# iacopo97/Multimodal-SAM-Adapter

Measured on AMD Instinct MI355X. Metric: images/sec encoder fwd @1024x1024 RGB+LiDAR ViT-L, higher is better.
Workload: dtype split-operand MFMA: fp16 hi + e5m2 cross terms (h8c / h8 planes, ViT / interaction / up-conv GEMMs) fp16 hi/lo pairs x3 (TwinConvNeXt: f3 planes) and bf16 hi/lo x3 (neck, head); attention blocks with the rel-pos terms fused: every contraction on one fp16 MFMA (q, k, v, P rounded to fp16) in the bloc

## Files before the change

include/mmsa.h:

```cpp
#ifndef MMSA_H
#define MMSA_H
#include <stddef.h>
#include <stdint.h>
#ifdef __cplusplus
extern "C" {
#endif

#ifdef MMSA_BUILDING_LIBRARY
typedef hipStream_t mmsa_stream_t;
#else
typedef void* mmsa_stream_t;
#endif

#include "mmsa_version.h"
int mmsa_version(void);
const char* mmsa_last_error(void);

int mmsa_debug_poison_lds(unsigned pattern, mmsa_stream_t stream);
int mmsa_event_create(void** ev);
int mmsa_event_record(void* ev, mmsa_stream_t stream);
int mmsa_event_elapsed_ms(void* start, void* stop, float* ms);
int mmsa_event_destroy(void* ev);

enum { MMSA_ACT_NONE = 0, MMSA_ACT_GELU = 1, MMSA_ACT_RELU = 2, MMSA_ACT_RELU6 = 3, MMSA_ACT_HSWISH = 4, MMSA_ACT_SIGMOID = 5 };

enum { MMSA_DT_F32 = 0, MMSA_DT_F16 = 1, MMSA_DT_F64 = 2 };

enum { MMSA_FMT_B3 = 0, MMSA_FMT_H8 = 1, MMSA_FMT_H8C = 2, MMSA_FMT_F3 = 3, MMSA_FMT_W8 = 4  };

int mmsa_ms_deform_attn_forward(const void* value, const int64_t* spatial_shapes, const int64_t* level_start_index,
                                const void* sampling_loc, const void* attn_weight, void* out, int batch,
                                int spatial_size, int num_heads, int channels, int num_levels, int num_query,
                                int num_point, int im2col_step, int dtype, mmsa_stream_t stream);

int mmsa_ms_deform_attn_backward(const void* value, const int64_t* spatial_shapes, const int64_t* level_start_index,
                                 const void* sampling_loc, const void* attn_weight, const void* grad_output,
                                 void* grad_value, void* grad_sampling_loc, void* grad_attn_weight, int batch,
                                 int spatial_size, int num_heads, int channels, int num_levels, int num_query,
                                 int num_point, int im2col_step, int dtype, mmsa_stream_t stream);

int mmsa_msda_fused(const float* value, const int64_t* spatial_shapes, const int64_t* level_start_index,
                    const float* raw, long ldraw, const float* ref_points, float* out, long ldo,
                    uint16_t* out_planes, long ldop , int out_fmt , int batch,
                    int spatial_size, int num_heads, int channels, int num_levels, int num_query, int num_point,
                    float* clamp_max , mmsa_stream_t stream);

int mmsa_msda_fused_planes(const uint16_t* value_planes, long ldvp, int lo_bytes, const int64_t* spatial_shapes, const int64_t* level_start_index,
                           const float* raw, long ldraw, const float* ref_points, float* out, long ldo,
                           uint16_t* out_planes, long ldop, int out_fmt, int batch,
                           int spatial_size, int num_heads, int channels, int num_levels, int num_query, int num_point,
                           float* clamp_max, mmsa_stream_t stream);

int mmsa_rowstats_finalize(const float* rowstats, int rows, int strips, int D, float eps, float* mean_rstd, mmsa_stream_t stream);

int mmsa_zero_bytes(void* p, size_t bytes, mmsa_stream_t stream);
int mmsa_gemm_split3(const float* A, const uint16_t* Ap, long lda, long strideA,
                     const uint16_t* Wp, long strideW,
                     const float* bias, long strideBias, const float* colscale, const float* resid, long ldr,
                     long strideR, int resid_mod, float beta, float* C, long ldc, long strideC,
                     uint16_t* Cp, long ldcp, long strideCp, int M, int N, int K,
                     int batch, int act, float alpha, int out_mode, int ps_H, int ps_W, int ps_C, int fmt, int cp_fmt,
                     int max_grid, float* rowstats_out, const float* rownorm_mean_rstd, const float* rownorm_colsum, int flavour,
                     float* clamp_max , mmsa_stream_t stream);

int mmsa_convnext_mlp_fused(const uint16_t* Ap, long lda, long strideA, const uint16_t* W1p, long strideW1, const uint16_t* W2p,
                            long strideW2, const float* b1, const float* b2, const float* gamma, float* x, long ldx, long strideX,
                            int M, int C, int batch, int max_grid, int fmt,
                            float* clamp_max , mmsa_stream_t stream);

int mmsa_split_planes(const float* src, long ld, int rows, int cols, int cols_pad, uint16_t* planes, int kind,
                      float* clamp_max , mmsa_stream_t stream);

int mmsa_attention(const float* qkv, long ldq, const float* qkv_bias, const float* rp, float* out, long ldo, int B,
                   int H, int W, int heads, int head_dim, int window_size, float scale, mmsa_stream_t stream);
int mmsa_attention_planes(const uint16_t* qkv_planes, long ldq, const uint16_t* bias_planes, const float* rp,
                          uint16_t* out_planes, long ldo, int B, int H, int W, int heads, int head_dim,
                          int window_size, float scale, int out_fmt ,
                          int v_fmt ,
                          float* max_abs_logit , mmsa_stream_t stream);

int mmsa_relpos_bias(const float* qkv, long ldq, const float* Rh, const float* Rw, float* rp, int B, int H, int W,
                     int heads, int head_dim, int window_size, mmsa_stream_t stream);
int mmsa_relpos_bias_planes(const uint16_t* qkv_planes, long ldq, const float* Rh, const float* Rw,
                            float* rp, int B, int H, int W, int heads, int head_dim, int window_size, mmsa_stream_t stream);

int mmsa_layernorm_rows(const float* x, long ldx, const float* w, const float* b, float eps, float* y, long ldy,
                        float* y2, long ldy2, uint16_t* y_planes, long ldp ,
                        int rows, int C, int map_mode, int map_H, int map_W, int group_rows, long w_gstride, long y_gcol,
                        int y_wrap, int plane_fmt , float* clamp_max ,
                        mmsa_stream_t stream);

int mmsa_colstats(const float* x, long ldx, long strideB, const float* wrow, int B, int HW, int C, double* out,
                  int out_is_zero , mmsa_stream_t stream);

int mmsa_ffrm_finalize(const double* stats, int B, int HW, int C, float mean_w, float mean_b, const float* Wc,
                       const float* gn_w, const float* gn_b, float* mean_o, float* rstd_o, float* mult_o,
                       float* scratch , mmsa_stream_t stream);
int mmsa_lnhw_apply(const float* x, long ldx, const float* mean, const float* rstd, const float* mult, const float* w,
                    const float* bias, float* y, long ldy, int B, int HW, int C, mmsa_stream_t stream);

int mmsa_dwconv_nhwc(const float* x, long ldx, long xstrideB, const float* w, const float* bias, float* y, long ldy,
                     long ystrideB, uint16_t* y_planes, long ldp, long pstrideB , int planes_fmt ,
                     int B, int H, int W, int C, int k, int act,
                     int imgs_per_group ,
                     float* rowstats ,
                     float* clamp_max , mmsa_stream_t stream);
int mmsa_gconv_nhwc(const float* x, long ldx, const float* w, const float* bias, float* y, long ldy, int B, int H,
                    int W, int G, int cin_g, int cout_g, int k, int act, mmsa_stream_t stream);
int mmsa_gfe_qkv_conv(const float* x, long ldx, const float* w, float* y, long ldy, int B, int H, int W, int G, int cin_g, int cout_g,
                      int* covered, mmsa_stream_t stream);
int mmsa_dwpair_gate(const float* x, long ldx, const float* w, float* y, long ldy, uint16_t* y_planes, long ldp, int B, int H,
                     int W, int C, mmsa_stream_t stream);
int mmsa_im2col_nchw(const float* x, int B, int Ctot, int c0, int Cin, int H, int W, int p, float* out, int Kpad,
                     mmsa_stream_t stream);

long mmsa_gram_tn_scratch_bytes(int B, int P, int c);
int mmsa_gram_tn(const float* X, long ldx, const float* Y, long ldy, long strideB, double* G , int B, int P, int c,
                 int nblk, void* scratch, long scratch_bytes, mmsa_stream_t stream);
int mmsa_chanattn_build(const double* G, const double* sq, long sq_strideB, const double* sk, long sk_strideB,
                        const float* temp, const float* Wp, uint16_t* planes , int B, int c, int cpad,
                        int heads, mmsa_stream_t stream);
// ... 136 lines not shown
```

multimodal-sam-adapter_amd/csrc/mlp_fused.hip:

```cpp
#include "common.h"

#define MF_GLDS16(gptr, lptr)                                                                               \
  __builtin_amdgcn_global_load_lds((const __attribute__((address_space(1))) void*)(gptr),                   \
                                   (__attribute__((address_space(3))) void*)(lptr), 16, 0, 0)

struct MlpFusedArgs {
  const unsigned short* Ap; long lda; long strideA;
  const unsigned short* W1p; long strideW1;
  const unsigned short* W2p; long strideW2;
  const float* b1; const float* b2; const float* gamma;
  float* x; long ldx; long strideX;
  int M, batch;
  int ntiles, tiles_per_batch;
  float* clamp;
};

#define MF_C 96
#define MF_HID (4 * MF_C)
#define MF_AS_BYTES (3 * 16384)
#define MF_SLOT 24576
#define MF_RING_OFF MF_AS_BYTES
#define MF_HS_OFF (MF_RING_OFF + 3 * MF_SLOT)
#define MF_BS_OFF (MF_HS_OFF + 32768)
#define MF_LDS (MF_BS_OFF + 8192)

template <bool F16>
__global__ __launch_bounds__(512, 1) void mlp_fused_kernel(MlpFusedArgs a) {
  float cw_ = 0.f;
  constexpr int C = MF_C, HID = MF_HID;
  constexpr int NSTEP = 2 * (HID / 64);
  constexpr int NT = C / 32;
  extern __shared__ __attribute__((aligned(16))) unsigned char smem[];
  unsigned char* As = smem;
  unsigned char* Hs = smem + MF_HS_OFF;
  float* Bs = reinterpret_cast<float*>(smem + MF_BS_OFF);
  for (int i = threadIdx.x; i < a.batch * HID; i += 512) Bs[i] = a.b1[i];
  const int tid = threadIdx.x, lane = tid & 63;
  const int wave = __builtin_amdgcn_readfirstlane(tid >> 6);
  const int wm = wave >> 1, wn = wave & 1;
  const int l15 = lane & 15, g = lane >> 4;
  const int drow = lane >> 3;
  const int dp_even = ((lane & 7) ^ (drow >> 1)) * 8;
  const int fslot = g ^ ((l15 >> 1) & 7);
  const int frag_hi = l15 * 128 + fslot * 16;
  const int frag_lo = l15 * 128 + (fslot ^ 4) * 16;
  const long w1_off = (long)(8 * wave + drow) * (2 * C) + ((wave & 1) ? (dp_even ^ 32) : dp_even);
  int w2_kb[3], w2_dst[3];
  long w2_off[3];
#pragma unroll
  for (int i = 0; i < 3; ++i) {
    const int p = wave + 8 * i, kb2 = p / 12, q = p - 12 * kb2;
    w2_kb[i] = kb2;
    w2_dst[i] = kb2 * 12288 + q * 1024;
    w2_off[i] = (long)(8 * q + drow) * (2 * HID) + ((q & 1) ? (dp_even ^ 32) : dp_even);
  }

  auto tile_of = [&](int tile, int& bz, int& m0) { bz = tile / a.tiles_per_batch; m0 = (tile - bz * a.tiles_per_batch) * 128; };
  auto issue_a = [&](int tile) {
    int bz, m0;
    tile_of(tile, bz, m0);
    const unsigned short* Ab = a.Ap + (long)bz * a.strideA;
#pragma unroll
    for (int i = 0; i < 6; ++i) {
      const int p = wave + 8 * i, kb = p >> 4, q = p & 15;
      const int row = min(m0 + 8 * q + drow, a.M - 1);
      MF_GLDS16(Ab + (long)row * a.lda + kb * 64 + ((q & 1) ? (dp_even ^ 32) : dp_even), As + kb * 16384 + q * 1024);
    }
  };
  auto issue = [&](int t, const unsigned short* W1b, const unsigned short* W2b, int slot) {
    unsigned char* sb = smem + MF_RING_OFF + slot * MF_SLOT;
    const int j = t >> 1;
    if ((t & 1) == 0) {
#pragma unroll
      for (int kb = 0; kb < 3; ++kb) MF_GLDS16(W1b + (long)j * 64 * (2 * C) + w1_off + kb * 64, sb + kb * 8192 + wave * 1024);
    } else {
#pragma unroll
      for (int i = 0; i < 3; ++i) MF_GLDS16(W2b + w2_off[i] + (2 * j + w2_kb[i]) * 64, sb + w2_dst[i]);
    }
  };

  int slot_c = 0;
  int tile = blockIdx.x;
  if (tile < a.ntiles) issue_a(tile);
  for (; tile < a.ntiles; tile += gridDim.x) {
    int bz, m0;
    tile_of(tile, bz, m0);
    const unsigned short* W1b = a.W1p + (long)bz * a.strideW1;
    const unsigned short* W2b = a.W2p + (long)bz * a.strideW2;
    f32x4 acc_o[2][NT];
#pragma unroll
    for (int mi = 0; mi < 2; ++mi)
#pragma unroll
      for (int nj = 0; nj < NT; ++nj) acc_o[mi][nj] = (f32x4){0.f, 0.f, 0.f, 0.f};
    f32x4 acc_h[2][2];
    issue(0, W1b, W2b, slot_c);
    issue(1, W1b, W2b, slot_c == 2 ? 0 : slot_c + 1);

#pragma unroll 1
    for (int t = 0; t < NSTEP; ++t) {
      if (t + 1 < NSTEP) asm volatile("s_waitcnt vmcnt(3)" ::: "memory");
      else asm volatile("s_waitcnt vmcnt(0)" ::: "memory");
      asm volatile("s_waitcnt lgkmcnt(0)" ::: "memory");
      __syncthreads();
      const unsigned char* sb = smem + MF_RING_OFF + slot_c * MF_SLOT;
      const int pf_slot = slot_c == 0 ? 2 : slot_c - 1;
      const int j = t >> 1;
      if ((t & 1) == 0) {
#pragma unroll
        for (int mi = 0; mi < 2; ++mi)
#pragma unroll
          for (int ni = 0; ni < 2; ++ni) acc_h[mi][ni] = (f32x4){0.f, 0.f, 0.f, 0.f};
#pragma unroll
        for (int kb = 0; kb < 3; ++kb) {
          bf16x8 ah[2], al[2], wh[2], wl[2];
#pragma unroll
          for (int i = 0; i < 2; ++i) {
            ah[i] = *reinterpret_cast<const bf16x8*>(As + kb * 16384 + (wm * 32 + i * 16) * 128 + frag_hi);
            al[i] = *reinterpret_cast<const bf16x8*>(As + kb * 16384 + (wm * 32 + i * 16) * 128 + frag_lo);
            wh[i] = *reinterpret_cast<const bf16x8*>(sb + kb * 8192 + (wn * 32 + i * 16) * 128 + frag_hi);
            wl[i] = *reinterpret_cast<const bf16x8*>(sb + kb * 8192 + (wn * 32 + i * 16) * 128 + frag_lo);
          }
#pragma unroll
          for (int mi = 0; mi < 2; ++mi)
#pragma unroll
            for (int ni = 0; ni < 2; ++ni) {
              acc_h[mi][ni] = (F16 ? __builtin_amdgcn_mfma_f32_16x16x32_f16(__builtin_bit_cast(f16x8, wl[ni]), __builtin_bit_cast(f16x8, ah[mi]), acc_h[mi][ni], 0, 0, 0) : __builtin_amdgcn_mfma_f32_16x16x32_bf16(wl[ni], ah[mi], acc_h[mi][ni], 0, 0, 0));
              acc_h[mi][ni] = (F16 ? __builtin_amdgcn_mfma_f32_16x16x32_f16(__builtin_bit_cast(f16x8, wh[ni]), __builtin_bit_cast(f16x8, al[mi]), acc_h[mi][ni], 0, 0, 0) : __builtin_amdgcn_mfma_f32_16x16x32_bf16(wh[ni], al[mi], acc_h[mi][ni], 0, 0, 0));
              acc_h[mi][ni] = (F16 ? __builtin_amdgcn_mfma_f32_16x16x32_f16(__builtin_bit_cast(f16x8, wh[ni]), __builtin_bit_cast(f16x8, ah[mi]), acc_h[mi][ni], 0, 0, 0) : __builtin_amdgcn_mfma_f32_16x16x32_bf16(wh[ni], ah[mi], acc_h[mi][ni], 0, 0, 0));
            }
        }
        if (t + 2 < NSTEP) issue(t + 2, W1b, W2b, pf_slot);
        const float* b1p = Bs + bz * HID + j * 64 + wn * 32;
#pragma unroll
        for (int ni = 0; ni < 2; ++ni) {
          const float4 bb = *reinterpret_cast<const float4*>(b1p + ni * 16 + 4 * g);
#pragma unroll
          for (int mi = 0; mi < 2; ++mi) {
            float4 o = make_float4(acc_h[mi][ni][0] + bb.x, acc_h[mi][ni][1] + bb.y, acc_h[mi][ni][2] + bb.z, acc_h[mi][ni][3] + bb.w);
            o = gelu4(o);
            uint2 hh, ll;
            if constexpr (F16) { clamp_see(cw_, o); f3_split4(o, hh, ll); } else split4(o, hh, ll);
            const int row = wm * 32 + mi * 16 + l15;
            const int chunk = ni * 2 + (g >> 1);
            const int sw = (row >> 1) & 7;
            unsigned char* rb = Hs + wn * 16384 + row * 128 + (g & 1) * 8;
            *reinterpret_cast<uint2*>(rb + ((chunk ^ sw) << 4)) = hh;
            *reinterpret_cast<uint2*>(rb + (((chunk + 4) ^ sw) << 4)) = ll;
          }
        }
      } else {
#pragma unroll
        for (int kb2 = 0; kb2 < 2; ++kb2) {
          bf16x8 ah[2], al[2];
#pragma unroll
          for (int i = 0; i < 2; ++i) {
            ah[i] = *reinterpret_cast<const bf16x8*>(Hs + kb2 * 16384 + (wm * 32 + i * 16) * 128 + frag_hi);
            al[i] = *reinterpret_cast<const bf16x8*>(Hs + kb2 * 16384 + (wm * 32 + i * 16) * 128 + frag_lo);
          }
#pragma unroll
          for (int nj = 0; nj < NT; ++nj) {
            const bf16x8 wh = *reinterpret_cast<const bf16x8*>(sb + kb2 * 12288 + (wn * (C / 2) + nj * 16) * 128 + frag_hi);
            const bf16x8 wl = *reinterpret_cast<const bf16x8*>(sb + kb2 * 12288 + (wn * (C / 2) + nj * 16) * 128 + frag_lo);
#pragma unroll
            for (int mi = 0; mi < 2; ++mi) {
              acc_o[mi][nj] = (F16 ? __builtin_amdgcn_mfma_f32_16x16x32_f16(__builtin_bit_cast(f16x8, wl), __builtin_bit_cast(f16x8, ah[mi]), acc_o[mi][nj], 0, 0, 0) : __builtin_amdgcn_mfma_f32_16x16x32_bf16(wl, ah[mi], acc_o[mi][nj], 0, 0, 0));
              acc_o[mi][nj] = (F16 ? __builtin_amdgcn_mfma_f32_16x16x32_f16(__builtin_bit_cast(f16x8, wh), __builtin_bit_cast(f16x8, al[mi]), acc_o[mi][nj], 0, 0, 0) : __builtin_amdgcn_mfma_f32_16x16x32_bf16(wh, al[mi], acc_o[mi][nj], 0, 0, 0));
              acc_o[mi][nj] = (F16 ? __builtin_amdgcn_mfma_f32_16x16x32_f16(__builtin_bit_cast(f16x8, wh), __builtin_bit_cast(f16x8, ah[mi]), acc_o[mi][nj], 0, 0, 0) : __builtin_amdgcn_mfma_f32_16x16x32_bf16(wh, ah[mi], acc_o[mi][nj], 0, 0, 0));
            }
          }
        }
        if (t + 2 < NSTEP) issue(t + 2, W1b, W2b, pf_slot);
        else if (t == NSTEP - 1 && tile + (int)gridDim.x < a.ntiles) issue_a(tile + gridDim.x);
      }
      slot_c = slot_c == 2 ? 0 : slot_c + 1;
    }

    float* xb = a.x + (long)bz * a.strideX;
    const float* b2p = a.b2 + (long)bz * C + wn * (C / 2);
    const float* gp = a.gamma + (long)bz * C + wn * (C / 2);
#pragma unroll
    for (int nj = 0; nj < NT; ++nj) {
      const float4 bb = *reinterpret_cast<const float4*>(b2p + nj * 16 + 4 * g);
      const float4 gg = *reinterpret_cast<const float4*>(gp + nj * 16 + 4 * g);
#pragma unroll
      for (int mi = 0; mi < 2; ++mi) {
        const int m = m0 + wm * 32 + mi * 16 + l15;
        if (m < a.M) {
          float* px = xb + (long)m * a.ldx + wn * (C / 2) + nj * 16 + 4 * g;
          const float4 rr = *reinterpret_cast<const float4*>(px);
          float4 o;
          o.x = rr.x + gg.x * (acc_o[mi][nj][0] + bb.x);
          o.y = rr.y + gg.y * (acc_o[mi][nj][1] + bb.y);
          o.z = rr.z + gg.z * (acc_o[mi][nj][2] + bb.z);
          o.w = rr.w + gg.w * (acc_o[mi][nj][3] + bb.w);
          *reinterpret_cast<float4*>(px) = o;
        }
      }
    }
  }
  if constexpr (F16) clamp_report(a.clamp, cw_, MMSA_F3_MAX);
}

extern "C" int mmsa_convnext_mlp_fused(const unsigned short* Ap, long lda, long strideA, const unsigned short* W1p, long strideW1,
                                       const unsigned short* W2p, long strideW2, const float* b1, const float* b2, const float* gamma,
                                       float* x, long ldx, long strideX, int M, int C, int batch, int max_grid, int fmt, float* clamp_max, hipStream_t stream) {
  MMSA_CHECK_ARG(Ap && W1p && W2p && b1 && b2 && gamma && x && M > 0 && batch > 0, "convnext_mlp_fused: bad args");
  MMSA_CHECK_ARG(C == MF_C, "convnext_mlp_fused: C = %d not supported (%d)", C, MF_C);
  MMSA_CHECK_ARG(fmt == MMSA_FMT_B3 || fmt == MMSA_FMT_F3, "convnext_mlp_fused: planes format %d (bf16 hi/lo or f3)", fmt);
  MMSA_CHECK_ARG((long)batch * 4 * C <= 2048, "convnext_mlp_fused: batch * 4C = %ld > 2048 (bias staging)", (long)batch * 4 * C);
  MMSA_CHECK_ARG(lda >= 2L * C && (lda & 63) == 0 && (strideA & 63) == 0 && (strideW1 & 63) == 0 && (strideW2 & 63) == 0,
                 "convnext_mlp_fused: plane strides must be multiples of 64");
  MMSA_CHECK_ARG(((((uintptr_t)Ap) | ((uintptr_t)W1p) | ((uintptr_t)W2p)) & 127) == 0, "convnext_mlp_fused: planes must be 128-byte aligned");
  MMSA_CHECK_ARG(((((uintptr_t)x) | ((uintptr_t)b1) | ((uintptr_t)b2) | ((uintptr_t)gamma)) & 15) == 0 && (ldx & 3) == 0 && (strideX & 3) == 0 && ldx >= C,
                 "convnext_mlp_fused: fp32 pointers must be 16-byte aligned, ldx %% 4 == 0");
  MlpFusedArgs a;
  a.Ap = Ap; a.lda = lda; a.strideA = strideA; a.W1p = W1p; a.strideW1 = strideW1; a.W2p = W2p; a.strideW2 = strideW2;
  a.b1 = b1; a.b2 = b2; a.gamma = gamma; a.x = x; a.ldx = ldx; a.strideX = strideX; a.M = M; a.batch = batch; a.clamp = clamp_max;
  a.tiles_per_batch = cdiv(M, 128);
  a.ntiles = a.tiles_per_batch * batch;
  static MmsaPerDevice per_dev_ = {};
  const int num_cus = mmsa_per_device(per_dev_, [] {
    (void)hipFuncSetAttribute((const void*)mlp_fused_kernel<false>, hipFuncAttributeMaxDynamicSharedMemorySize, MF_LDS);
    (void)hipFuncSetAttribute((const void*)mlp_fused_kernel<true>, hipFuncAttributeMaxDynamicSharedMemorySize, MF_LDS);
  });
  const int cus = (max_grid > 0 && max_grid < num_cus) ? max_grid : num_cus;
  const int grid = a.ntiles < cus ? a.ntiles : cus;
  if (fmt == MMSA_FMT_F3) hipLaunchKernelGGL(mlp_fused_kernel<true>, dim3(grid), dim3(512), MF_LDS, stream, a);
  else hipLaunchKernelGGL(mlp_fused_kernel<false>, dim3(grid), dim3(512), MF_LDS, stream, a);
  MMSA_CHECK_LAUNCH("convnext_mlp_fused");
  return MMSA_OK;
}
```

multimodal-sam-adapter_amd/mmsa/backbone.py:

```python
import contextlib
import functools
import math
import os

import torch
import torch.nn as nn

from . import ops, pack
from .pack import PackPlan, _linear_resize_rows, fold_gfe_qkv
from .params import CONVNEXT_ARCH, build_tree

_VIT_DEFAULTS = dict(img_size=1024, patch_size=16, in_chans=3, embed_dim=1024, depth=24, mlp_ratio=4.0,
                     qkv_bias=True, use_abs_pos=True, use_rel_pos=True, rel_pos_zero_init=True, window_size=14,
                     global_attn_indexes=[5, 11, 17, 23], pretrained_size=1024, fix=False)


class OperandRangeError(RuntimeError):
    """A forward converted a value beyond the range of an fp16-based operand format (the clamp watch word, include/mmsa.h) and nothing is left to
    re-route: `range_fallback` is off, or the value is a q / k / v (or a qkv bias / rel-pos table entry) beyond +-65504 inside the attention kernels,
    which read fp16-based planes in every mode.  The outputs of that forward are invalid."""


class Workspace:

# ... 690 lines not shown
            for i in range(4):
                self._taps[f"twin{i}"] = tcat[i].clone()
        offs = [0, 0, sizes[1][0] * sizes[1][1], sizes[1][0] * sizes[1][1] + sizes[2][0] * sizes[2][1]]
        joins = []
        for i in range(4):
            sn = s_neck[i]
            sn.wait_event(ev_x[i])
            with torch.cuda.stream(sn):
                if i == 0:
                    self._neck_level(0, pk["neck"][0], tcat[0], B, sizes[0][0], sizes[0][1], chans[0], c1_out, 0, tcat_p[0])
                else:
                    self._neck_level(i, pk["neck"][i], tcat[i], B, sizes[i][0], sizes[i][1], chans[i], cbuf[offs[i]:], Nc * D, tcat_p[i])
                e = torch.cuda.Event()
                e.record(sn)
                joins.append(e)
        if not join:
            return joins
        for e in joins[1:]:
            main.wait_event(e)
        return joins[0]

    def _twin_batched(self, x, B, sizes, tcat, stage_events, tcat_p=None):
        pk, ws = self._packed, self._ws
        chans = self.channels
        st = pk["twin2"]
        t = "cnb_"
        h0, w0 = sizes[0]
        P0 = B * h0 * w0
        kp = st["stem"].kpad
        a = ws.get(t + "stem_a", 2 * P0, kp)
        for si in range(2):
            ops.im2col_nchw(x, 3 * si, 3, 4, a[si * P0:(si + 1) * P0])
        t0 = ws.get(t + "tmp", 2 * P0, chans[0])
        ops.gemm(a, st["stem"], t0, bias=st["stem_b"], batch=2, m=P0, stride_a=P0 * kp, stride_w=st["stem"].n * 2 * kp,
                 stride_bias=chans[0], stride_c=P0 * chans[0])
        cur = ws.get(t + "cur0", 2 * P0, chans[0])
        ops.layernorm(t0, st["stem_nw"], st["stem_nb"], 1e-6, cur, group_rows=P0, w_gstride=chans[0])
        for i in range(4):
            hh, wwd = sizes[i]
            P = B * hh * wwd
            c = chans[i]
            if i >= 1:
                ds = st["ds"][i - 1]
                cp = chans[i - 1]
                Pp = B * sizes[i - 1][0] * sizes[i - 1][1]
                pa = ws.planes(t + "patch", 2 * P, 4 * cp, fmt=ds["w"].fmt)
                ops.layernorm(cur, ds["nw"], ds["nb"], 1e-6, out_planes=pa, patchify=(sizes[i - 1][0], sizes[i - 1][1]),
                              group_rows=Pp, w_gstride=cp)
                cur = ws.get(t + f"cur{i}", 2 * P, c)
                ops.gemm(pa, ds["w"], cur, bias=ds["b"], batch=2, m=P, stride_a=P * 2 * pa.kpad, stride_w=ds["w"].n * 2 * ds["w"].kpad,
                         stride_bias=c, stride_c=P * c)
            d = ws.get(t + "tmp", 2 * P, c)
            wf = st["stages"][i][0]["pw1"].fmt
            n = ws.planes(t + "n", 2 * P, c, fmt=wf)
            hbuf = ws.planes(t + "h", 2 * P, 4 * c, fmt=st["stages"][i][0]["pw2"].fmt)
            fuse_mlp = ops.convnext_mlp_fused_supported(c) and bool(getattr(self, "fuse_convnext_mlp", True))
            fold = "pw1f" in st["stages"][i][0] and not fuse_mlp and hh % 8 == 0 and wwd % 8 == 0 and P >= 128
            if fold:
                rs = ws.get(t + "rs", 2 * P, 2 * (c // 64))
                mr = ws.get(t + "mr", 2 * P, 2)
            for blk in st["stages"][i]:
                if fold:
                    ops.dwconv(cur, blk["dw"], blk["dw_b"], None, 2 * B, hh, wwd, 7, imgs_per_group=B, out_planes=n, rowstats_out=rs)
                    ops.rowstats_finalize(rs, 2 * P, c, 1e-6, mr)
                    ops.gemm(n, blk["pw1f"], bias=blk["pw1_bf"], act="gelu", out_planes=hbuf, row_norm=(mr, blk["pw1_cs"]), batch=2, m=P,
                             stride_a=P * 2 * n.kpad, stride_w=blk["pw1f"].n * 2 * blk["pw1f"].kpad, stride_bias=4 * c, stride_cp=P * 2 * hbuf.kpad)
                    ops.gemm(hbuf, blk["pw2"], cur, bias=blk["pw2_b"], colscale=blk["gamma"], resid=cur, batch=2, m=P,
                             stride_a=P * 2 * hbuf.kpad, stride_w=blk["pw2"].n * 2 * blk["pw2"].kpad, stride_bias=c,
                             stride_r=P * c, stride_c=P * c)
                    continue
                ops.dwconv(cur, blk["dw"], blk["dw_b"], d, 2 * B, hh, wwd, 7, imgs_per_group=B)
                ops.layernorm(d, blk["nw"], blk["nb"], 1e-6, out_planes=n, group_rows=P, w_gstride=c)
                if fuse_mlp:
                    ops.convnext_mlp_fused(n, blk["pw1"], blk["pw2"], blk["pw1_b"], blk["pw2_b"], blk["gamma"], cur, P, batch=2,
                                           stride_a=P * 2 * n.kpad, stride_w1=blk["pw1"].n * 2 * blk["pw1"].kpad,
                                           stride_w2=blk["pw2"].n * 2 * blk["pw2"].kpad, stride_x=P * c)
                    continue
                ops.gemm(n, blk["pw1"], bias=blk["pw1_b"], act="gelu", out_planes=hbuf, batch=2, m=P, stride_a=P * 2 * n.kpad,
                         stride_w=blk["pw1"].n * 2 * blk["pw1"].kpad, stride_bias=4 * c, stride_cp=hbuf.batch_stride(P))
                ops.gemm(hbuf, blk["pw2"], cur, bias=blk["pw2_b"], colscale=blk["gamma"], resid=cur, batch=2, m=P,
                         stride_a=hbuf.batch_stride(P), stride_w=blk["pw2"].batch_stride(blk["pw2"].n), stride_bias=c,
                         stride_r=P * c, stride_c=P * c)
            nw, nb = st["out_norm"][i]
            ops.layernorm(cur, nw, nb, 1e-6, tcat[i], group_rows=P, w_gstride=c, y_gcol=c, y_wrap=True,
                          out_planes=tcat_p[i] if tcat_p is not None else None)
            ev = torch.cuda.Event()
            ev.record(torch.cuda.current_stream())
            stage_events.append(ev)

    def _neck_level(self, level, lv, t, B, h, w, c, out, out_stride_b, tp=None):
        ws = _Tagged(self._ws, f"nk{level}_")
        C = 2 * c
        HW = h * w
        P = B * HW
        gcat = ws.get("nk_g", P, C)
        lcat = ws.get("nk_l", P, C)
        pl_ok = tp is not None and c % 32 == 0
        gcat_p = ws.planes("nk_gp", P, C) if pl_ok else None
        lcat_p = ws.planes("nk_lp", P, C) if pl_ok else None
        n_st, n_g, n_st2 = B * 3 * 3 * c, B * c * c, B * 3 * C
        acc_blk = ws.get("nk_acc", 1, 2 * (n_st + n_g) + n_g + n_st2, dtype=torch.float64)
        ops.zero_(acc_blk[0, :2 * n_st + n_st2])
        gram_scr = ws.get("nk_gscr", 1, (ops.gram_tn_scratch_bytes(B, HW, c) + 3) // 4)
        acc_off = [0, 2 * n_st + n_st2]

        def acc_buf(rows, cols, gram=False):
            o = acc_off[int(gram)]
            acc_off[int(gram)] = o + rows * cols
            return acc_blk[0, o:o + rows * cols].view(rows, cols)
        for m in range(2):
            X = t[:, m * c:(m + 1) * c]
            gp = lv["gfe"][m]
            y = ws.get("nk_y", P, c)
            s = ws.get("nk_s", P, c)
            ops.layernorm(X, gp["nw"], gp["nb"], 1e-5, y, out2=s)
            q2 = ws.get("nk_q2", P, 3 * c)
            if not ("q12" in gp and getattr(self, "fuse_gfe_qkv", True) and ops.gfe_qkv(y, gp["q12"], q2, B, h, w, 32, c // 32, 3 * c // 32)):
                q1 = ws.get("nk_q1", P, 3 * c)
                ops.gconv(y, gp["q1"], None, q1, B, h, w, 32, c // 32, 3 * c // 32, 1)
                ops.gconv(q1, gp["q2"], None, q2, B, h, w, 32, 3 * c // 32, 3 * c // 32, 3)
            st = acc_buf(B * 3, 3 * c)
            ops.colstats(q2, HW * 3 * c, B, HW, st, out_is_zero=True)
            g = acc_buf(B * c, c, gram=True)
            ops.gram_tn(q2[:, :c], q2[:, c:2 * c], HW * 3 * c, g, B, HW, nblk=8, scratch=gram_scr)
# ... 125 lines not shown
```

multimodal-sam-adapter_amd/mmsa/lib.py:

```python
import ctypes
import os
from ctypes import c_char_p, c_double, c_float, c_int, c_long, c_void_p, POINTER

_HERE = os.path.dirname(os.path.abspath(__file__))
LIB_PATH = os.environ.get("MMSA_LIB") or os.path.join(_HERE, "libmmsa_hip.so")

if not os.path.exists(LIB_PATH):
    raise RuntimeError(
        f"{LIB_PATH} not found: the MI355X HIP library is required (no CPU/PyTorch fallback exists). "
        "Build it with: python multimodal-sam-adapter_amd/build.py")

import torch

_lib = ctypes.CDLL(LIB_PATH)

P = c_void_p
I = c_int
L = c_long
F = c_float

_PAINT_TAIL = [P, I, P, I, I, I, I, I, P, P, I, I, c_double, c_double, c_double, c_double, P, P]
SIGNATURES = {
    "mmsa_version": [],
    "mmsa_last_error": [],
    "mmsa_debug_poison_lds": [ctypes.c_uint, P],
    "mmsa_event_create": [POINTER(c_void_p)],
    "mmsa_event_record": [P, P],
    "mmsa_event_elapsed_ms": [P, P, POINTER(c_float)],
    "mmsa_event_destroy": [P],
    "mmsa_ms_deform_attn_forward": [P, P, P, P, P, P, I, I, I, I, I, I, I, I, I, P],
    "mmsa_ms_deform_attn_backward": [P, P, P, P, P, P, P, P, P, I, I, I, I, I, I, I, I, I, P],
    "mmsa_msda_fused": [P, P, P, P, L, P, P, L, P, L, I, I, I, I, I, I, I, I, P, P],
    "mmsa_msda_fused_planes": [P, L, I, P, P, P, L, P, P, L, P, L, I, I, I, I, I, I, I, I, P, P],
    "mmsa_gemm_split3": [P, P, L, L, P, L, P, L, P, P, L, L, I, F, P, L, L, P, L, L, I, I, I, I, I, F, I, I, I, I, I, I, I, P, P, P, I, P, P],
    "mmsa_convnext_mlp_fused": [P, L, L, P, L, P, L, P, P, P, P, L, L, I, I, I, I, I, P, P],
    "mmsa_rowstats_finalize": [P, I, I, I, F, P, P],
    "mmsa_zero_bytes": [P, ctypes.c_size_t, P],
    "mmsa_split_planes": [P, L, I, I, I, P, I, P, P],
    "mmsa_attention": [P, L, P, P, P, L, I, I, I, I, I, I, F, P],
    "mmsa_attention_planes": [P, L, P, P, P, L, I, I, I, I, I, I, F, I, I, P, P],
    "mmsa_relpos_bias": [P, L, P, P, P, I, I, I, I, I, I, P],
    "mmsa_relpos_bias_planes": [P, L, P, P, P, I, I, I, I, I, I, P],
    "mmsa_layernorm_rows": [P, L, P, P, F, P, L, P, L, P, L, I, I, I, I, I, I, L, L, I, I, P, P],
    "mmsa_colstats": [P, L, L, P, I, I, I, P, I, P],
    "mmsa_ffrm_finalize": [P, I, I, I, F, F, P, P, P, P, P, P, P, P],
    "mmsa_lnhw_apply": [P, L, P, P, P, P, P, P, L, I, I, I, P],
    "mmsa_dwconv_nhwc": [P, L, L, P, P, P, L, L, P, L, L, I, I, I, I, I, I, I, I, P, P, P],
    "mmsa_dwpair_gate": [P, L, P, P, L, P, L, I, I, I, I, P],
    "mmsa_gconv_nhwc": [P, L, P, P, P, L, I, I, I, I, I, I, I, I, P],
    "mmsa_gfe_qkv_conv": [P, L, P, P, L, I, I, I, I, I, I, POINTER(c_int), P],
    "mmsa_im2col_nchw": [P, I, I, I, I, I, I, I, P, I, P],
    "mmsa_gram_tn": [P, L, P, L, L, P, I, I, I, I, P, L, P],
    "mmsa_gram_tn_scratch_bytes": [I, I, I],
    "mmsa_chanattn_build": [P, P, L, P, L, P, P, P, I, I, I, I, P],
    "mmsa_gffm_build": [P, P, P, I, I, I, P],
    "mmsa_gelu_gate": [P, L, P, L, L, I, P],
    "mmsa_pool_hw": [P, L, P, L, I, I, I, I, P],
    "mmsa_ca_apply": [P, L, P, L, P, L, P, L, I, I, I, I, P],
    "mmsa_tail_fuse": [P, L, L, P, L, P, P, P, P, L, I, I, I, I, I, I, P],
    "mmsa_global_attention_planes": [P, L, P, P, P, L, I, I, I, I, I, F, I, I, P, P],
    "mmsa_window_attention_planes": [P, L, P, P, P, P, L, I, I, I, I, I, I, F, I, I, P, P],
    "mmsa_nchw_to_planes": [P, L, P, L, I, I, L, P],
    "mmsa_head_fuse": [P, P, I, I, P, I, I, P, I, I, L, P, P, P, L, P, L, I, I, I, I, I, P],
    "mmsa_tokens_to_nchw": [P, L, P, I, L, I, P],
    "mmsa_bilinear_accum_nchw": [P, L, I, I, I, I, P, I, I, I, I, I, I, P, I, P],
    "mmsa_div_count_nchw": [P, P, I, I, L, P],
    "mmsa_argmax_nchw": [P, P, I, I, L, P],
    "mmsa_crop_batch_nchw": [P, I, I, I, I, P, I, P, I, I, P],
    "mmsa_slide_argmax": [P, I, I, I, I, P, P, I, I, I, I, I, P, P],
    "mmsa_slide_argmax_resized": [P, I, I, I, I, P, P, I, I, I, I, I, I, I, I, I, P, P],
    "mmsa_softmax_flip_accum_nchw": [P, P, I, I, I, I, I, I, I, P],
    "mmsa_aug_argmax": [P, P, I, I, P, P, I, P, I, I, I, P, P],
    "mmsa_argmax_max_nchw": [P, P, P, I, I, L, P],
    "mmsa_slide_argmax_conf": [P, I, I, I, I, P, P, P, I, I, I, I, I, P, P],
    "mmsa_slide_argmax_resized_conf": [P, I, I, I, I, P, P, P, I, I, I, I, I, I, I, I, I, P, P],
    "mmsa_aug_argmax_conf": [P, P, I, I, P, P, I, P, P, I, I, I, P, P],
    "mmsa_preprocess_nhwc": [P, I, P, I, I, I, I, P, P, P, P, P, P, I, I, P],
    "mmsa_preprocess_crops": [P, I, P, I, I, I, I, P, P, P, P, P, I, I, P, I, P, I, I, P],
    "mmsa_preprocess_resize_nhwc": [P, I, P, I, I, I, I, P, P, P, P, P, P, I, I, I, I, P, P, P, P, I, P],
    "mmsa_preprocess_resize_crops": [P, I, P, I, I, I, I, P, P, P, P, P, I, I, P, I, P, I, I, I, I, P, P, P, P, I, P],
    "mmsa_eval_confusion_u8": [P, P, I, I, I, I, I, P, I, P, P, P, I, P, P],
    "mmsa_eval_calibration": [P, P, P, I, I, I, I, I, P, I, P, P, P, I, I, P, P],
    "mmsa_eval_selective": [P, P, P, I, I, I, I, I, P, I, P, P, P, I, I, P, P],
    "mmsa_abstain_u8": [P, P, L, I, I, P, P],
    "mmsa_slide_argmax_conf_t": [P, I, I, I, I, P, P, P, I, I, I, I, I, P, F, P],
    "mmsa_slide_argmax_resized_conf_t": [P, I, I, I, I, P, P, P, I, I, I, I, I, I, I, I, I, P, F, P],
    "mmsa_softmax_flip_accum_nchw_t": [P, P, I, I, I, I, I, I, I, F, P],
    "mmsa_temperature_sweep_nchw": [P, P, I, I, I, I, I, I, P, P, P, P, I, P, I, I, P, P],
# ... 49 lines not shown
```

multimodal-sam-adapter_amd/mmsa/ops.py:

```python
import ctypes

import os

import torch

from . import lib

ACT = {"none": 0, "gelu": 1, "relu": 2, "relu6": 3, "hswish": 4, "sigmoid": 5}

GEMM_PROFILE = None
CLAMP_WATCH = None
GEMM_MAX_GRID = 0
GEMM_FLAVOUR = 0
GEMM_SHAPES = None


def _event():
    ev = ctypes.c_void_p()
    lib.call("mmsa_event_create", ctypes.byref(ev))
    return ev


def collect_gemm_profile(prof):
    flops, ms = 0.0, 0.0
# ... 249 lines not shown


def gemm(a, w, out=None, bias=None, act="none", alpha=1.0, colscale=None, resid=None, beta=1.0, resid_mod=0,
         batch=1, stride_a=0, stride_w=0, stride_bias=0, stride_r=0, stride_c=0, m=None, pixel_shuffle=None,
         out_planes=None, stride_cp=0, rowstats_out=None, row_norm=None):
    fmt = w.fmt
    if isinstance(a, Planes):
        pap, ma, ka, lda = a.mat("A")
        pa = None
        if ka < w.kpad:
            raise RuntimeError(f"mmsa.gemm: A planes have {ka} columns but the packed weight expects K={w.kpad}")
        if a.fmt != w.afmt or a.weight or (w.fmt == FMT_H8 and not w.weight) or (w.fmt == FMT_H8C and w.weight):
            raise RuntimeError(f"mmsa.gemm: operand formats differ (A fmt {a.fmt}, W fmt {w.fmt} weight={w.weight})")
    elif fmt not in (FMT_B3, FMT_F3):
        raise RuntimeError("mmsa.gemm: h8 weights need A as h8 planes")
    else:
        pa, ma, ka, lda = _mat(a, "A")
        pap = None
        if ka < w.kpad and lda < w.kpad:
            raise RuntimeError(f"mmsa.gemm: A has {ka} columns (ld {lda}) but the packed weight expects K={w.kpad}")
    m = ma if m is None else m
    pc, ldc = None, 0
    if out is not None:
        pc, _, _, ldc = _mat(out, "C")
    pcp, ldcp = None, 0
    if out_planes is not None:
        pcp, _, _, ldcp = out_planes.mat("Cplanes")
    pr, ldr = None, 0
    if resid is not None:
        pr, _, _, ldr = _mat(resid, "resid")
    ps = pixel_shuffle or (0, 0, 0)
    prof = GEMM_PROFILE
    if prof is not None:
        e0, e1 = _event(), _event()
        lib.call("mmsa_event_record", e0, _stream())
    lib.call("mmsa_gemm_split3", pa, pap, lda, stride_a, w.p.data_ptr(), stride_w,
             _chk(bias, name="bias"), stride_bias, _chk(colscale, name="colscale"), pr, ldr, stride_r, resid_mod, beta,
             pc, ldc, stride_c, pcp, ldcp, stride_cp, m, w.n, w.kpad, batch, ACT[act], alpha,
             1 if pixel_shuffle else 0, ps[0], ps[1], ps[2], fmt, cp_format(out_planes), GEMM_MAX_GRID,
             _chk(rowstats_out), _chk(row_norm[0]) if row_norm else None, _chk(row_norm[1]) if row_norm else None, GEMM_FLAVOUR, _clamp_ptr(), _stream())
    if prof is not None:
        lib.call("mmsa_event_record", e1, _stream())
        ob = 3.0 if fmt in (FMT_H8C, FMT_W8) else 4.0
        wb = 1.0 if fmt == FMT_W8 else ob
        pb = 0.0 if out_planes is None else (3.0 if out_planes.fmt == FMT_H8C else 4.0)
        prof.append((2.0 * m * w.n * w.k * batch, e0, e1,
                     batch * (ob * m * w.kpad + wb * w.n * w.kpad + m * w.n * (pb + 4.0 * ((1 if out is not None else 0) + (1 if resid is not None else 0))))))
        if GEMM_SHAPES is not None:
            GEMM_SHAPES.append((m, w.n, w.k, batch, act, resid is not None, ("C" if out is not None else "") + ("P" if out_planes is not None else ""),
                                "planes" if pap is not None else "fp32"))
    return out if out is not None else out_planes


def convnext_mlp_fused(a, w1, w2, b1, b2, gamma, x, m, batch=1, stride_a=0, stride_w1=0, stride_w2=0, stride_x=0):
    pa, _, _, lda = a.mat("A")
    px, _, c, ldx = _mat(x, "x")
    if a.fmt not in (FMT_B3, FMT_F3) or w1.fmt != a.fmt or w2.fmt != a.fmt:
        raise RuntimeError("mmsa.convnext_mlp_fused: bf16 hi/lo or f3 planes expected, the same format for A, W1 and W2")
    prof = GEMM_PROFILE
    if prof is not None:
        e0, e1 = _event(), _event()
        lib.call("mmsa_event_record", e0, _stream())
    lib.call("mmsa_convnext_mlp_fused", pa, lda, stride_a, w1.p.data_ptr(), stride_w1, w2.p.data_ptr(), stride_w2, _chk(b1), _chk(b2),
             _chk(gamma), px, ldx, stride_x, m, c, batch, GEMM_MAX_GRID, a.fmt, _clamp_ptr(), _stream())
    if prof is not None:
        lib.call("mmsa_event_record", e1, _stream())
        prof.append((2.0 * 2.0 * m * c * 4 * c * batch, e0, e1, 4.0 * batch * (m * c * 3 + 2 * 4 * c * c)))
        if GEMM_SHAPES is not None:
            GEMM_SHAPES.append((m, c, 4 * c, batch, "gelu", True, "C", "fused-pair"))
    return x


def convnext_mlp_fused_supported(c):
    return c == 96


def zero_(t):
    if not t.is_contiguous():
        raise RuntimeError("mmsa.ops.zero_: contiguous tensor expected")
    if t.numel():
        lib.call("mmsa_zero_bytes", _chk(t, t.dtype), t.numel() * t.element_size(), _stream())
    return t


def rowstats_finalize(rowstats, rows, d, eps, out):
    lib.call("mmsa_rowstats_finalize", _chk(rowstats), rows, d // 64, d, eps, _chk(out), _stream())
    return out


def layernorm(x, w, b, eps, out=None, out2=None, patchify=None, out_planes=None, group_rows=0, w_gstride=0, y_gcol=0, y_wrap=False):
    px, rows, c, ldx = _mat(x, "x")
    py, ldy = None, 0
    if out is not None:
        py, _, _, ldy = _mat(out, "y")
    p2, ld2 = None, 0
    if out2 is not None:
        p2, _, _, ld2 = _mat(out2, "y2")
    pp, ldp = None, 0
    if out_planes is not None:
        pp, _, _, ldp = out_planes.mat("y planes")
    mh, mw = patchify or (0, 0)
    lib.call("mmsa_layernorm_rows", px, ldx, _chk(w), _chk(b), eps, py, ldy, p2, ld2, pp, ldp, rows, c,
             1 if patchify else 0, mh, mw, group_rows, w_gstride, y_gcol, 1 if y_wrap else 0,
             out_planes.fmt if out_planes is not None else FMT_B3, _clamp_ptr(), _stream())
    return out if out is not None else out_planes


MSDA_DTYPES = {torch.float32: 0, torch.float16: 1, torch.float64: 2}


def _msda_args(value, spatial_shapes, level_start_index, sampling_loc, attn_weight, extra=()):
    dt = value.dtype
    if dt not in MSDA_DTYPES:
        raise RuntimeError(f"ms_deform_attn: dtype {dt} not supported (float32, float16, float64)")
    for t, n in ((value, "value"), (sampling_loc, "sampling_loc"), (attn_weight, "attn_weight")) + tuple(extra):
        if not t.is_contiguous():
            raise RuntimeError(f"{n} tensor has to be contiguous")
# ... 306 lines not shown
```

Measured before the change: 67.41.

## Fuse ConvNeXt LayerNorm into the fused MLP kernel's A-tile staging

```diff
diff --git a/include/mmsa.h b/include/mmsa.h
--- a/include/mmsa.h
+++ b/include/mmsa.h
@@ -67,6 +67,11 @@
                             long strideW2, const float* b1, const float* b2, const float* gamma, float* x, long ldx, long strideX,
                             int M, int C, int batch, int max_grid, int fmt,
                             float* clamp_max , mmsa_stream_t stream);
+
+int mmsa_convnext_mlp_fused_ln(const float* D, long ldd, long strideD, const float* ln_w, const float* ln_b, float eps, const uint16_t* W1p,
+                               long strideW1, const uint16_t* W2p, long strideW2, const float* b1, const float* b2, const float* gamma, float* x,
+                               long ldx, long strideX, int M, int C, int batch, int max_grid, int fmt,
+                               float* clamp_max , mmsa_stream_t stream);
 
 int mmsa_split_planes(const float* src, long ld, int rows, int cols, int cols_pad, uint16_t* planes, int kind,
                       float* clamp_max , mmsa_stream_t stream);
diff --git a/multimodal-sam-adapter_amd/csrc/mlp_fused.hip b/multimodal-sam-adapter_amd/csrc/mlp_fused.hip
--- a/multimodal-sam-adapter_amd/csrc/mlp_fused.hip
+++ b/multimodal-sam-adapter_amd/csrc/mlp_fused.hip
@@ -13,7 +13,13 @@
   int M, batch;
   int ntiles, tiles_per_batch;
   float* clamp;
+  const float* D; long ldd; long strideD;
+  const float* lnw; const float* lnb; float eps;
 };
+
+#define MF_MFMA(w_, a_, c_)                                                                                                                   \
+  (F16 ? __builtin_amdgcn_mfma_f32_16x16x32_f16(__builtin_bit_cast(f16x8, w_), __builtin_bit_cast(f16x8, a_), c_, 0, 0, 0) \
+       : __builtin_amdgcn_mfma_f32_16x16x32_bf16(w_, a_, c_, 0, 0, 0))
 
 #define MF_C 96
 #define MF_HID (4 * MF_C)
@@ -24,7 +30,7 @@
 #define MF_BS_OFF (MF_HS_OFF + 32768)
 #define MF_LDS (MF_BS_OFF + 8192)
 
-template <bool F16>
+template <bool F16, bool LN>
 __global__ __launch_bounds__(512, 1) void mlp_fused_kernel(MlpFusedArgs a) {
   float cw_ = 0.f;
   constexpr int C = MF_C, HID = MF_HID;
@@ -67,6 +73,62 @@
       MF_GLDS16(Ab + (long)row * a.lda + kb * 64 + ((q & 1) ? (dp_even ^ 32) : dp_even), As + kb * 16384 + q * 1024);
     }
   };
+  float4 dn[2][3], lw[3], lb[3];
+  auto load_d = [&](int tile) {
+    int bz, m0;
+    tile_of(tile, bz, m0);
+    const float* Db = a.D + (long)bz * a.strideD + 4 * (lane & 7);
+    const float* wb = a.lnw + (long)bz * C + 4 * (lane & 7);
+    const float* bb = a.lnb + (long)bz * C + 4 * (lane & 7);
+#pragma unroll
+    for (int ps = 0; ps < 2; ++ps) {
+      const int row = min(m0 + 16 * wave + 8 * ps + drow, a.M - 1);
+#pragma unroll
+      for (int kb = 0; kb < 3; ++kb) dn[ps][kb] = *reinterpret_cast<const float4*>(Db + (long)row * a.ldd + kb * 32);
+    }
+#pragma unroll
+    for (int kb = 0; kb < 3; ++kb) {
+      lw[kb] = *reinterpret_cast<const float4*>(wb + kb * 32);
+      lb[kb] = *reinterpret_cast<const float4*>(bb + kb * 32);
+    }
+  };
+  auto row8_sum = [](float v) {
+#pragma unroll
+    for (int o = 4; o > 0; o >>= 1) v += __shfl_xor(v, o, 64);
+    return v;
+  };
+  auto write_a = [&]() {
+#pragma unroll
+    for (int ps = 0; ps < 2; ++ps) {
+      float s = 0.f;
+#pragma unroll
+      for (int kb = 0; kb < 3; ++kb) s += (dn[ps][kb].x + dn[ps][kb].y) + (dn[ps][kb].z + dn[ps][kb].w);
+      const float mean = row8_sum(s) / (float)C;
+      float q = 0.f;
+#pragma unroll
+      for (int kb = 0; kb < 3; ++kb) {
+        const float dx = dn[ps][kb].x - mean, dy = dn[ps][kb].y - mean, dz = dn[ps][kb].z - mean, dw = dn[ps][kb].w - mean;
+        q += (dx * dx + dy * dy) + (dz * dz + dw * dw);
+      }
+      const float rstd = 1.0f / sqrtf(row8_sum(q) / (float)C + a.eps);
+      const int row = 16 * wave + 8 * ps + drow;
+      const int sw = (row >> 1) & 7;
+      const int chunk = (lane & 7) >> 1;
+      unsigned char* rb = As + row * 128 + (lane & 1) * 8;
+#pragma unroll
+      for (int kb = 0; kb < 3; ++kb) {
+        float4 o;
+        o.x = (dn[ps][kb].x - mean) * rstd * lw[kb].x + lb[kb].x;
+        o.y = (dn[ps][kb].y - mean) * rstd * lw[kb].y + lb[kb].y;
+        o.z = (dn[ps][kb].z - mean) * rstd * lw[kb].z + lb[kb].z;
+        o.w = (dn[ps][kb].w - mean) * rstd * lw[kb].w + lb[kb].w;
+        uint2 hh, ll;
+        if constexpr (F16) { clamp_see(cw_, o); f3_split4(o, hh, ll); } else split4(o, hh, ll);
+        *reinterpret_cast<uint2*>(rb + kb * 16384 + ((chunk ^ sw) << 4)) = hh;
+        *reinterpret_cast<uint2*>(rb + kb * 16384 + (((chunk + 4) ^ sw) << 4)) = ll;
+      }
+    }
+  };
   auto issue = [&](int t, const unsigned short* W1b, const unsigned short* W2b, int slot) {
     unsigned char* sb = smem + MF_RING_OFF + slot * MF_SLOT;
     const int j = t >> 1;
@@ -81,7 +143,9 @@
 
   int slot_c = 0;
   int tile = blockIdx.x;
-  if (tile < a.ntiles) issue_a(tile);
+  if (tile < a.ntiles) {
+    if constexpr (LN) { load_d(tile); write_a(); } else issue_a(tile);
+  }
   for (; tile < a.ntiles; tile += gridDim.x) {
     int bz, m0;
     tile_of(tile, bz, m0);
@@ -106,6 +170,9 @@
       const int pf_slot = slot_c == 0 ? 2 : slot_c - 1;
       const int j = t >> 1;
       if ((t & 1) == 0) {
+        if constexpr (LN) {
+          if (t == NSTEP - 2 && tile + (int)gridDim.x < a.ntiles) load_d(tile + gridDim.x);
+        }
 #pragma unroll
         for (int mi = 0; mi < 2; ++mi)
 #pragma unroll
@@ -124,9 +191,9 @@
           for (int mi = 0; mi < 2; ++mi)
 #pragma unroll
             for (int ni = 0; ni < 2; ++ni) {
-              acc_h[mi][ni] = (F16 ? __builtin_amdgcn_mfma_f32_16x16x32_f16(__builtin_bit_cast(f16x8, wl[ni]), __builtin_bit_cast(f16x8, ah[mi]), acc_h[mi][ni], 0, 0, 0) : __builtin_amdgcn_mfma_f32_16x16x32_bf16(wl[ni], ah[mi], acc_h[mi][ni], 0, 0, 0));
-              acc_h[mi][ni] = (F16 ? __builtin_amdgcn_mfma_f32_16x16x32_f16(__builtin_bit_cast(f16x8, wh[ni]), __builtin_bit_cast(f16x8, al[mi]), acc_h[mi][ni], 0, 0, 0) : __builtin_amdgcn_mfma_f32_16x16x32_bf16(wh[ni], al[mi], acc_h[mi][ni], 0, 0, 0));
-              acc_h[mi][ni] = (F16 ? __builtin_amdgcn_mfma_f32_16x16x32_f16(__builtin_bit_cast(f16x8, wh[ni]), __builtin_bit_cast(f16x8, ah[mi]), acc_h[mi][ni], 0, 0, 0) : __builtin_amdgcn_mfma_f32_16x16x32_bf16(wh[ni], ah[mi], acc_h[mi][ni], 0, 0, 0));
+              acc_h[mi][ni] = MF_MFMA(wl[ni], ah[mi], acc_h[mi][ni]);
+              acc_h[mi][ni] = MF_MFMA(wh[ni], al[mi], acc_h[mi][ni]);
+              acc_h[mi][ni] = MF_MFMA(wh[ni], ah[mi], acc_h[mi][ni]);
             }
         }
         if (t + 2 < NSTEP) issue(t + 2, W1b, W2b, pf_slot);
@@ -163,14 +230,16 @@
             const bf16x8 wl = *reinterpret_cast<const bf16x8*>(sb + kb2 * 12288 + (wn * (C / 2) + nj * 16) * 128 + frag_lo);
 #pragma unroll
             for (int mi = 0; mi < 2; ++mi) {
-              acc_o[mi][nj] = (F16 ? __builtin_amdgcn_mfma_f32_16x16x32_f16(__builtin_bit_cast(f16x8, wl), __builtin_bit_cast(f16x8, ah[mi]), acc_o[mi][nj], 0, 0, 0) : __builtin_amdgcn_mfma_f32_16x16x32_bf16(wl, ah[mi], acc_o[mi][nj], 0, 0, 0));
-              acc_o[mi][nj] = (F16 ? __builtin_amdgcn_mfma_f32_16x16x32_f16(__builtin_bit_cast(f16x8, wh), __builtin_bit_cast(f16x8, al[mi]), acc_o[mi][nj], 0, 0, 0) : __builtin_amdgcn_mfma_f32_16x16x32_bf16(wh, al[mi], acc_o[mi][nj], 0, 0, 0));
-              acc_o[mi][nj] = (F16 ? __builtin_amdgcn_mfma_f32_16x16x32_f16(__builtin_bit_cast(f16x8, wh), __builtin_bit_cast(f16x8, ah[mi]), acc_o[mi][nj], 0, 0, 0) : __builtin_amdgcn_mfma_f32_16x16x32_bf16(wh, ah[mi], acc_o[mi][nj], 0, 0, 0));
+              acc_o[mi][nj] = MF_MFMA(wl, ah[mi], acc_o[mi][nj]);
+              acc_o[mi][nj] = MF_MFMA(wh, al[mi], acc_o[mi][nj]);
+              acc_o[mi][nj] = MF_MFMA(wh, ah[mi], acc_o[mi][nj]);
             }
           }
         }
         if (t + 2 < NSTEP) issue(t + 2, W1b, W2b, pf_slot);
-        else if (t == NSTEP - 1 && tile + (int)gridDim.x < a.ntiles) issue_a(tile + gridDim.x);
+        else if (t == NSTEP - 1 && tile + (int)gridDim.x < a.ntiles) {
+          if constexpr (LN) write_a(); else issue_a(tile + gridDim.x);
+        }
       }
       slot_c = slot_c == 2 ? 0 : slot_c + 1;
     }
@@ -199,6 +268,23 @@
     }
   }
   if constexpr (F16) clamp_report(a.clamp, cw_, MMSA_F3_MAX);
+}
+
+template <bool LN>
+static int mlp_fused_launch(MlpFusedArgs& a, int fmt, int max_grid, hipStream_t stream) {
+  a.tiles_per_batch = cdiv(a.M, 128);
+  a.ntiles = a.tiles_per_batch * a.batch;
+  static MmsaPerDevice per_dev_ = {};
+  const int num_cus = mmsa_per_device(per_dev_, [] {
+    (void)hipFuncSetAttribute((const void*)mlp_fused_kernel<false, LN>, hipFuncAttributeMaxDynamicSharedMemorySize, MF_LDS);
+    (void)hipFuncSetAttribute((const void*)mlp_fused_kernel<true, LN>, hipFuncAttributeMaxDynamicSharedMemorySize, MF_LDS);
+  });
+  const int cus = (max_grid > 0 && max_grid < num_cus) ? max_grid : num_cus;
+  const int grid = a.ntiles < cus ? a.ntiles : cus;
+  if (fmt == MMSA_FMT_F3) hipLaunchKernelGGL((mlp_fused_kernel<true, LN>), dim3(grid), dim3(512), MF_LDS, stream, a);
+  else hipLaunchKernelGGL((mlp_fused_kernel<false, LN>), dim3(grid), dim3(512), MF_LDS, stream, a);
+  MMSA_CHECK_LAUNCH("convnext_mlp_fused");
+  return MMSA_OK;
 }
 
 extern "C" int mmsa_convnext_mlp_fused(const unsigned short* Ap, long lda, long strideA, const unsigned short* W1p, long strideW1,
@@ -213,20 +299,29 @@
   MMSA_CHECK_ARG(((((uintptr_t)Ap) | ((uintptr_t)W1p) | ((uintptr_t)W2p)) & 127) == 0, "convnext_mlp_fused: planes must be 128-byte aligned");
   MMSA_CHECK_ARG(((((uintptr_t)x) | ((uintptr_t)b1) | ((uintptr_t)b2) | ((uintptr_t)gamma)) & 15) == 0 && (ldx & 3) == 0 && (strideX & 3) == 0 && ldx >= C,
                  "convnext_mlp_fused: fp32 pointers must be 16-byte aligned, ldx %% 4 == 0");
-  MlpFusedArgs a;
+  MlpFusedArgs a = {};
   a.Ap = Ap; a.lda = lda; a.strideA = strideA; a.W1p = W1p; a.strideW1 = strideW1; a.W2p = W2p; a.strideW2 = strideW2;
   a.b1 = b1; a.b2 = b2; a.gamma = gamma; a.x = x; a.ldx = ldx; a.strideX = strideX; a.M = M; a.batch = batch; a.clamp = clamp_max;
-  a.tiles_per_batch = cdiv(M, 128);
-  a.ntiles = a.tiles_per_batch * batch;
-  static MmsaPerDevice per_dev_ = {};
-  const int num_cus = mmsa_per_device(per_dev_, [] {
-    (void)hipFuncSetAttribute((const void*)mlp_fused_kernel<false>, hipFuncAttributeMaxDynamicSharedMemorySize, MF_LDS);
-    (void)hipFuncSetAttribute((const void*)mlp_fused_kernel<true>, hipFuncAttributeMaxDynamicSharedMemorySize, MF_LDS);
-  });
-  const int cus = (max_grid > 0 && max_grid < num_cus) ? max_grid : num_cus;
-  const int grid = a.ntiles < cus ? a.ntiles : cus;
-  if (fmt == MMSA_FMT_F3) hipLaunchKernelGGL(mlp_fused_kernel<true>, dim3(grid), dim3(512), MF_LDS, stream, a);
-  else hipLaunchKernelGGL(mlp_fused_kernel<false>, dim3(grid), dim3(512), MF_LDS, stream, a);
-  MMSA_CHECK_LAUNCH("convnext_mlp_fused");
-  return MMSA_OK;
+  return mlp_fused_launch<false>(a, fmt, max_grid, stream);
 }
+
+extern "C" int mmsa_convnext_mlp_fused_ln(const float* D, long ldd, long strideD, const float* ln_w, const float* ln_b, float eps,
+                                          const unsigned short* W1p, long strideW1, const unsigned short* W2p, long strideW2, const float* b1, const float* b2,
+                                          const float* gamma, float* x, long ldx, long strideX, int M, int C, int batch, int max_grid, int fmt,
+                                          float* clamp_max, hipStream_t stream) {
+  MMSA_CHECK_ARG(D && ln_w && ln_b && W1p && W2p && b1 && b2 && gamma && x && M > 0 && batch > 0, "convnext_mlp_fused_ln: bad args");
+  MMSA_CHECK_ARG(C == MF_C, "convnext_mlp_fused_ln: C = %d not supported (%d)", C, MF_C);
+  MMSA_CHECK_ARG(fmt == MMSA_FMT_B3 || fmt == MMSA_FMT_F3, "convnext_mlp_fused_ln: planes format %d (bf16 hi/lo or f3)", fmt);
+  MMSA_CHECK_ARG((long)batch * 4 * C <= 2048, "convnext_mlp_fused_ln: batch * 4C = %ld > 2048 (bias staging)", (long)batch * 4 * C);
+  MMSA_CHECK_ARG((strideW1 & 63) == 0 && (strideW2 & 63) == 0, "convnext_mlp_fused_ln: plane strides must be multiples of 64");
+  MMSA_CHECK_ARG(((((uintptr_t)W1p) | ((uintptr_t)W2p)) & 127) == 0, "convnext_mlp_fused_ln: planes must be 128-byte aligned");
+  MMSA_CHECK_ARG(((((uintptr_t)x) | ((uintptr_t)b1) | ((uintptr_t)b2) | ((uintptr_t)gamma)) & 15) == 0 && (ldx & 3) == 0 && (strideX & 3) == 0 && ldx >= C,
+                 "convnext_mlp_fused_ln: fp32 pointers must be 16-byte aligned, ldx %% 4 == 0");
+  MMSA_CHECK_ARG(((((uintptr_t)D) | ((uintptr_t)ln_w) | ((uintptr_t)ln_b)) & 15) == 0 && (ldd & 3) == 0 && (strideD & 3) == 0 && ldd >= C,
+                 "convnext_mlp_fused_ln: D, ln_w, ln_b must be 16-byte aligned, ldd %% 4 == 0");
+  MlpFusedArgs a = {};
+  a.D = D; a.ldd = ldd; a.strideD = strideD; a.lnw = ln_w; a.lnb = ln_b; a.eps = eps;
+  a.W1p = W1p; a.strideW1 = strideW1; a.W2p = W2p; a.strideW2 = strideW2;
+  a.b1 = b1; a.b2 = b2; a.gamma = gamma; a.x = x; a.ldx = ldx; a.strideX = strideX; a.M = M; a.batch = batch; a.clamp = clamp_max;
+  return mlp_fused_launch<true>(a, fmt, max_grid, stream);
+}
diff --git a/multimodal-sam-adapter_amd/mmsa/backbone.py b/multimodal-sam-adapter_amd/mmsa/backbone.py
--- a/multimodal-sam-adapter_amd/mmsa/backbone.py
+++ b/multimodal-sam-adapter_amd/mmsa/backbone.py
@@ -766,9 +766,10 @@
                          stride_bias=c, stride_c=P * c)
             d = ws.get(t + "tmp", 2 * P, c)
             wf = st["stages"][i][0]["pw1"].fmt
-            n = ws.planes(t + "n", 2 * P, c, fmt=wf)
+            fuse_mlp = ops.convnext_mlp_fused_supported(c) and bool(getattr(self, "fuse_convnext_mlp", True))
+            fuse_ln = fuse_mlp and bool(getattr(self, "fuse_convnext_ln", True))
+            n = None if fuse_ln else ws.planes(t + "n", 2 * P, c, fmt=wf)
             hbuf = ws.planes(t + "h", 2 * P, 4 * c, fmt=st["stages"][i][0]["pw2"].fmt)
-            fuse_mlp = ops.convnext_mlp_fused_supported(c) and bool(getattr(self, "fuse_convnext_mlp", True))
             fold = "pw1f" in st["stages"][i][0] and not fuse_mlp and hh % 8 == 0 and wwd % 8 == 0 and P >= 128
             if fold:
                 rs = ws.get(t + "rs", 2 * P, 2 * (c // 64))
@@ -784,6 +785,11 @@
                              stride_r=P * c, stride_c=P * c)
                     continue
                 ops.dwconv(cur, blk["dw"], blk["dw_b"], d, 2 * B, hh, wwd, 7, imgs_per_group=B)
+                if fuse_ln:
+                    ops.convnext_mlp_fused(None, blk["pw1"], blk["pw2"], blk["pw1_b"], blk["pw2_b"], blk["gamma"], cur, P, batch=2,
+                                           stride_w1=blk["pw1"].n * 2 * blk["pw1"].kpad, stride_w2=blk["pw2"].n * 2 * blk["pw2"].kpad, stride_x=P * c,
+                                           ln=(d, blk["nw"], blk["nb"], 1e-6), stride_d=P * c)
+                    continue
                 ops.layernorm(d, blk["nw"], blk["nb"], 1e-6, out_planes=n, group_rows=P, w_gstride=c)
                 if fuse_mlp:
                     ops.convnext_mlp_fused(n, blk["pw1"], blk["pw2"], blk["pw1_b"], blk["pw2_b"], blk["gamma"], cur, P, batch=2,
diff --git a/multimodal-sam-adapter_amd/mmsa/lib.py b/multimodal-sam-adapter_amd/mmsa/lib.py
--- a/multimodal-sam-adapter_amd/mmsa/lib.py
+++ b/multimodal-sam-adapter_amd/mmsa/lib.py
@@ -34,6 +34,7 @@
     "mmsa_msda_fused_planes": [P, L, I, P, P, P, L, P, P, L, P, L, I, I, I, I, I, I, I, I, P, P],
     "mmsa_gemm_split3": [P, P, L, L, P, L, P, L, P, P, L, L, I, F, P, L, L, P, L, L, I, I, I, I, I, F, I, I, I, I, I, I, I, P, P, P, I, P, P],
     "mmsa_convnext_mlp_fused": [P, L, L, P, L, P, L, P, P, P, P, L, L, I, I, I, I, I, P, P],
+    "mmsa_convnext_mlp_fused_ln": [P, L, L, P, P, F, P, L, P, L, P, P, P, P, L, L, I, I, I, I, I, P, P],
     "mmsa_rowstats_finalize": [P, I, I, I, F, P, P],
     "mmsa_zero_bytes": [P, ctypes.c_size_t, P],
     "mmsa_split_planes": [P, L, I, I, I, P, I, P, P],
diff --git a/multimodal-sam-adapter_amd/mmsa/ops.py b/multimodal-sam-adapter_amd/mmsa/ops.py
--- a/multimodal-sam-adapter_amd/mmsa/ops.py
+++ b/multimodal-sam-adapter_amd/mmsa/ops.py
@@ -325,17 +325,31 @@
     return out if out is not None else out_planes
 
 
-def convnext_mlp_fused(a, w1, w2, b1, b2, gamma, x, m, batch=1, stride_a=0, stride_w1=0, stride_w2=0, stride_x=0):
-    pa, _, _, lda = a.mat("A")
+def convnext_mlp_fused(a, w1, w2, b1, b2, gamma, x, m, batch=1, stride_a=0, stride_w1=0, stride_w2=0, stride_x=0, ln=None, stride_d=0):
     px, _, c, ldx = _mat(x, "x")
-    if a.fmt not in (FMT_B3, FMT_F3) or w1.fmt != a.fmt or w2.fmt != a.fmt:
+    if ln is None:
+        pa, _, _, lda = a.mat("A")
+        fmt = a.fmt
+    else:
+        if a is not None:
+            raise RuntimeError("mmsa.convnext_mlp_fused: give either the planes `a` or ln=(d, w, b, eps)")
+        d, ln_w, ln_b, eps = ln
+        pd, _, cd, ldd = _mat(d, "d")
+        if cd != c:
+            raise RuntimeError(f"mmsa.convnext_mlp_fused: d has {cd} channels, x has {c}")
+        fmt = w1.fmt
+    if fmt not in (FMT_B3, FMT_F3) or w1.fmt != fmt or w2.fmt != fmt:
         raise RuntimeError("mmsa.convnext_mlp_fused: bf16 hi/lo or f3 planes expected, the same format for A, W1 and W2")
     prof = GEMM_PROFILE
     if prof is not None:
         e0, e1 = _event(), _event()
         lib.call("mmsa_event_record", e0, _stream())
-    lib.call("mmsa_convnext_mlp_fused", pa, lda, stride_a, w1.p.data_ptr(), stride_w1, w2.p.data_ptr(), stride_w2, _chk(b1), _chk(b2),
-             _chk(gamma), px, ldx, stride_x, m, c, batch, GEMM_MAX_GRID, a.fmt, _clamp_ptr(), _stream())
+    if ln is None:
+        lib.call("mmsa_convnext_mlp_fused", pa, lda, stride_a, w1.p.data_ptr(), stride_w1, w2.p.data_ptr(), stride_w2, _chk(b1), _chk(b2),
+                 _chk(gamma), px, ldx, stride_x, m, c, batch, GEMM_MAX_GRID, fmt, _clamp_ptr(), _stream())
+    else:
+        lib.call("mmsa_convnext_mlp_fused_ln", pd, ldd, stride_d, _chk(ln_w), _chk(ln_b), eps, w1.p.data_ptr(), stride_w1, w2.p.data_ptr(), stride_w2,
+                 _chk(b1), _chk(b2), _chk(gamma), px, ldx, stride_x, m, c, batch, GEMM_MAX_GRID, fmt, _clamp_ptr(), _stream())
     if prof is not None:
         lib.call("mmsa_event_record", e1, _stream())
         prof.append((2.0 * 2.0 * m * c * 4 * c * batch, e0, e1, 4.0 * batch * (m * c * 3 + 2 * 4 * c * c)))
```

Measured after the change: 67.74, median of 6. About the same (+0.5%).
